# natalieklein/gpcsd

Measured on AMD Instinct MI355X. Metric: gpcsd_loglik_plus_predict_trials_per_sec, higher is better.
Workload: dtype f64; 1 GPU; GPCSD2D 384ch x 500t x 50 trials/GPU, fp64, ngl 20x60 (BASELINE cfg3/cfg4); n_elec=384, n_t=500, trials_per_gpu=50, total_trials=50, parallelism=trial-sharded x1, next_step_announced=True

## Files before the change

### gpcsd_amd/csrc/ctx.hpp

```cpp
#pragma once
#include <hip/hip_runtime.h>

#include <cstdarg>
#include <cstdio>
#include <cstring>
#include <map>
#include <string>
#include <vector>

#include "../../include/gpcsd_hip.h"

namespace gpcsd {

struct HipError {
    int code;
    std::string msg;
};

#define GP_HIP(expr)                                                                          \
    do {                                                                                      \
        hipError_t _e = (expr);                                                               \
        if (_e != hipSuccess) {                                                               \
            char _b[512];                                                                     \
            snprintf(_b, sizeof(_b), "%s:%d: %s -> %s", __FILE__, __LINE__, #expr,            \
// ... 41 lines not shown
        if (done[d]) return false;
        done[d] = true;
        return true;
    }
};
}

struct PredSink;
struct PairLl;
struct PredCall {
    const gpcsd_hparams *hp = nullptr;
    const double *z = nullptr, *tstar = nullptr;
    int nz = 0, ntstar = 0, type = 0;
    bool want_lists = false, async = false;
    PredSink *sink = nullptr;
    int solve_pass = 0;
    PairLl *ll = nullptr;
    bool prelude_side = false;
};

struct gpcsd_ctx {
    int device = 0;
    hipStream_t stream = nullptr;
    hipStream_t stream2 = nullptr;
    hipStream_t stream3 = nullptr;
    hipStream_t stream4 = nullptr;
    hipStream_t stream5 = nullptr;
    static constexpr int SCAL_N = 64, STATUS_N = 8, STATUS_LATE = 4;
    static constexpr int RESULT_DOUBLES = SCAL_N + STATUS_N / 2;
    double *h_result = nullptr;
    bool capturing = false;
// ... 323 lines not shown
```

### gpcsd_amd/csrc/gram.hip

```cpp
#include "devutil.hpp"
#include "kernels.hpp"

namespace gpcsd {

template <typename T>
__device__ __forceinline__ T dev_b_fwd_1d(T r, T R) {
    const T q = (r / R) * (r / R);
    return sqrt(q + T(1)) - sqrt(q);
}

template <typename T>
__device__ __forceinline__ T dev_b_fwd_2d_w(T w, T R, T eps) {
    const T re = R + eps;
    return log(re + sqrt(re * re + w * w)) - log(eps + sqrt(eps * eps + w * w));
}

__global__ void b_fwd_1d_kernel(const double *__restrict__ r, long n, double R, double *__restrict__ out) {
    for (long i = blockIdx.x * (long)blockDim.x + threadIdx.x; i < n; i += (long)gridDim.x * blockDim.x)
        out[i] = dev_b_fwd_1d<double>(r[i], R);
}

__global__ void b_fwd_2d_kernel(const double *__restrict__ d1, const double *__restrict__ d2, const double *__restrict__ w,
                                long n, double R, double eps, double *__restrict__ out) {
    for (long i = blockIdx.x * (long)blockDim.x + threadIdx.x; i < n; i += (long)gridDim.x * blockDim.x) {
// ... 362 lines not shown
                const double lg = (lane < nk) ? log(mypiv) : 0.0;
                logsum += wave_sum(lg);
            }
            __builtin_amdgcn_wave_barrier();
            if (k0 + LT_CK < np) store_chunk(buf ^ 1);
        }
        quad += wave_sum(lane < nr ? q : 0.0);
    }
    if (lane == 0) {
        g.partials[item] = quad;
        g.partials[nitems + item] = logsum;
    }
}

constexpr int LS_CPL = 4;
typedef double dbl2_t __attribute__((ext_vector_type(2)));
__global__ __launch_bounds__(64 * LT_WAVES) void ll_tridiag_scan_kernel(LlTridiagArgs g) {
    __shared__ double tile[LT_WAVES][2][64][LT_CK + 1];
    __shared__ dbl2_t coef[LT_WAVES][64 * LS_CPL + LT_CK];
    __shared__ double pexc[LT_WAVES][64 * LS_CPL + 1];
    const int lane = threadIdx.x & 63, wid = __builtin_amdgcn_readfirstlane(threadIdx.x >> 6);
    const int item = blockIdx.x * LT_WAVES + wid, nitems = 2 * g.nx;
    if (item >= nitems) return;
    const int xr = item >> 1, p = item & 1;
    const int np = g.np[p];
    if (np <= 0) {
        if (lane == 0) {
            g.partials[item] = 0.0;
            g.partials[nitems + item] = 0.0;
        }
        return;
    }
    const double lam_m = g.es[xr] * g.amax[p][0], sig = g.sig[0];
    const double *__restrict__ dd = g.d[p], *__restrict__ ee = g.e[p];
    const double *__restrict__ Wx = g.W + (long)xr * g.R * g.nt + g.c0[p];
    const int half = lane >> 5, kk_l = lane & 31;
    double stg[LT_RPL];
    auto load_chunk = [&](int r0, int nr, int k0) {
        const int nk = min(LT_CK, np - k0);
#pragma unroll
        for (int i = 0; i < LT_RPL; ++i) {
            const int rr = half + 2 * i;
            stg[i] = (rr < nr && kk_l < nk) ? Wx[(long)(r0 + rr) * g.nt + k0 + kk_l] : 0.0;
        }
    };
    auto store_chunk = [&](int buf) {
#pragma unroll
        for (int i = 0; i < LT_RPL; ++i) tile[wid][buf][half + 2 * i][kk_l] = stg[i];
    };
    load_chunk(0, min(64, g.R), 0);
    double logsum;
    {
        double a[LS_CPL], b2[LS_CPL], bb[LS_CPL];
#pragma unroll
        for (int cc = 0; cc < LS_CPL; ++cc) {
            const int k = lane * LS_CPL + cc;
            a[cc] = (k < np) ? lam_m * dd[k] + sig : 1.0;
            bb[cc] = (k >= 1 && k < np) ? lam_m * ee[k - 1] : 0.0;
            b2[cc] = bb[cc] * bb[cc];
        }
        auto renorm = [](double &x0, double &x1, double &x2, double &x3) {
            const double big = fmax(fmax(fabs(x0), fabs(x1)), fmax(fabs(x2), fabs(x3)));
            int ex;
            (void)frexp(big, &ex);
            x0 = ldexp(x0, -ex); x1 = ldexp(x1, -ex); x2 = ldexp(x2, -ex); x3 = ldexp(x3, -ex);
        };
        double m00 = a[0], m01 = -b2[0], m10 = 1.0, m11 = 0.0;
#pragma unroll
        for (int cc = 1; cc < LS_CPL; ++cc) {
            const double n00 = a[cc] * m00 - b2[cc] * m10, n01 = a[cc] * m01 - b2[cc] * m11;
            m10 = m00; m11 = m01; m00 = n00; m01 = n01;
        }
        renorm(m00, m01, m10, m11);
#pragma unroll
        for (int dlt = 1; dlt < 64; dlt <<= 1) {
            const double e00 = __shfl_up(m00, dlt), e01 = __shfl_up(m01, dlt), e10 = __shfl_up(m10, dlt), e11 = __shfl_up(m11, dlt);
            if (lane >= dlt) {
                double n00 = m00 * e00 + m01 * e10, n01 = m00 * e01 + m01 * e11;
                double n10 = m10 * e00 + m11 * e10, n11 = m10 * e01 + m11 * e11;
                renorm(n00, n01, n10, n11);
                m00 = n00; m01 = n01; m10 = n10; m11 = n11;
            }
        }
        double t0 = __shfl_up(m00, 1), t1 = __shfl_up(m10, 1);
        if (lane == 0) { t0 = 1.0; t1 = 0.0; }
        double pv[LS_CPL];
#pragma unroll
        for (int cc = 0; cc < LS_CPL; ++cc) {
            const double tn = a[cc] * t0 - b2[cc] * t1;
            pv[cc] = t0 / tn;
            t1 = t0; t0 = tn;
            if (cc == 1) {
                int ex;
                (void)frexp(t0, &ex);
                t0 = ldexp(t0, -ex); t1 = ldexp(t1, -ex);
            }
        }
#pragma unroll
        for (int cc = 0; cc < LS_CPL; ++cc) pexc[wid][lane * LS_CPL + cc + 1] = pv[cc];
        if (lane == 0) pexc[wid][0] = 0.0;
        __builtin_amdgcn_wave_barrier();
        {
            double gk[LS_CPL], rk[LS_CPL], G = 1.0, H = 0.0;
#pragma unroll
            for (int cc = 0; cc < LS_CPL; ++cc) {
                const double pl = pexc[wid][lane * LS_CPL + cc];
                const double sk = fma(-b2[cc], pl, a[cc]);
                rk[cc] = fma(-pv[cc], sk, 1.0);
                gk[cc] = b2[cc] * pl * pv[cc];
                H = fma(gk[cc], H, -rk[cc]);
                G *= gk[cc];
            }
#pragma unroll
            for (int dlt = 1; dlt < 64; dlt <<= 1) {
                const double Ge = __shfl_up(G, dlt), He = __shfl_up(H, dlt);
                if (lane >= dlt) {
                    H = fma(G, He, H);
                    G *= Ge;
                }
            }
            double eta = __shfl_up(H, 1);
            if (lane == 0) eta = 0.0;
#pragma unroll
            for (int cc = 0; cc < LS_CPL; ++cc) {
                eta = fma(gk[cc], eta, -rk[cc]);
                pv[cc] = fma(-pv[cc], eta, pv[cc]);
            }
            __builtin_amdgcn_wave_barrier();
#pragma unroll
            for (int cc = 0; cc < LS_CPL; ++cc) pexc[wid][lane * LS_CPL + cc + 1] = pv[cc];
            __builtin_amdgcn_wave_barrier();
        }
        double dk[LS_CPL], lg = 0.0;
#pragma unroll
        for (int cc = 0; cc < LS_CPL; ++cc) {
            const int k = lane * LS_CPL + cc;
            dk[cc] = a[cc] - b2[cc] * pexc[wid][k];
            pv[cc] = 1.0 / dk[cc];
            if (k < np) lg += log(dk[cc]);
        }
        logsum = wave_sum(lg);
        __builtin_amdgcn_wave_barrier();
#pragma unroll
        for (int cc = 0; cc < LS_CPL; ++cc) pexc[wid][lane * LS_CPL + cc + 1] = pv[cc];
        __builtin_amdgcn_wave_barrier();
#pragma unroll
        for (int cc = 0; cc < LS_CPL; ++cc) {
            const int k = lane * LS_CPL + cc;
            dbl2_t cf;
            cf.x = (k < np) ? bb[cc] * pexc[wid][k] : 0.0;
            cf.y = (k < np) ? pv[cc] : 0.0;
            coef[wid][k] = cf;
        }
        if (lane < LT_CK) coef[wid][64 * LS_CPL + lane] = dbl2_t{0.0, 0.0};
    }
    double quad = 0.0;
    for (int r0 = 0; r0 < g.R; r0 += 64) {
        const int nr = min(64, g.R - r0);
        if (r0 > 0) load_chunk(r0, nr, 0);
        __builtin_amdgcn_wave_barrier();
        store_chunk(0);
        double z = 0.0, q[4] = {0.0, 0.0, 0.0, 0.0};
        int buf = 0;
        for (int k0 = 0; k0 < np; k0 += LT_CK, buf ^= 1) {
            if (k0 + LT_CK < np) load_chunk(r0, nr, k0 + LT_CK);
            __builtin_amdgcn_wave_barrier();
            double wv[LT_CK];
            dbl2_t cf[LT_CK];
#pragma unroll
            for (int kk = 0; kk < LT_CK; ++kk) {
                wv[kk] = tile[wid][buf][lane][kk];
                cf[kk] = coef[wid][k0 + kk];
            }
#pragma unroll
            for (int kk = 0; kk < LT_CK; ++kk) {
                z = fma(-cf[kk].x, z, wv[kk]);
                q[kk & 3] = fma(z * z, cf[kk].y, q[kk & 3]);
            }
            __builtin_amdgcn_wave_barrier();
            if (k0 + LT_CK < np) store_chunk(buf ^ 1);
        }
        quad += wave_sum(lane < nr ? (q[0] + q[1]) + (q[2] + q[3]) : 0.0);
    }
    if (lane == 0) {
        g.partials[item] = quad;
        g.partials[nitems + item] = logsum;
    }
}

__global__ __launch_bounds__(256) void ll_tridiag_reduce_kernel(const double *__restrict__ partials, int nitems, double *out_sumlog,
                                                                double *out_quad, double *host_slot, const double *status_src,
                                                                int status_at, int status_doubles) {
    __shared__ double sh[256];
    const double *p = partials + (blockIdx.x == 0 ? nitems : 0);
    double s = 0.0;
    for (int i = threadIdx.x; i < nitems; i += 256) s += p[i];
    sh[threadIdx.x] = s;
    __syncthreads();
    for (int w = 128; w > 0; w >>= 1) {
        if ((int)threadIdx.x < w) sh[threadIdx.x] += sh[threadIdx.x + w];
// ... 21 lines not shown
                  double *out_sumlog, double *out_quad, hipStream_t s, double *host_slot, const double *status_src, int status_at,
                  int status_doubles, int variant) {
    LlTridiagArgs g{};
    g.W = W; g.es = es; g.sig = sig; g.nx = nx; g.R = R; g.nt = nt;
    for (int p = 0; p < 2; ++p) {
        g.d[p] = d[p]; g.e[p] = e[p]; g.amax[p] = amax[p]; g.np[p] = np[p]; g.c0[p] = c0[p];
    }
    const int nitems = 2 * nx;
    g.partials = c->buf<double>("ll_tridiag_partials", (size_t)2 * nitems);
    ProfScope ps(c, "ll_tridiag", 0.0, s);
    static const bool serial_env = getenv("GPCSD_LL_PIVOT_SCAN") && getenv("GPCSD_LL_PIVOT_SCAN")[0] == '0';
    const bool serial = variant ? variant == 1 : serial_env;
    GP_REQUIRE(variant != 2 || std::max(np[0], np[1]) <= 64 * LS_CPL, -3, "ll_tridiag: the scan kernel takes blocks of at most %d columns",
               64 * LS_CPL);
    if (!serial && std::max(np[0], np[1]) <= 64 * LS_CPL)
        hipLaunchKernelGGL(ll_tridiag_scan_kernel, dim3(ceil_div(nitems, LT_WAVES)), dim3(64 * LT_WAVES), 0, s, g);
    else
        hipLaunchKernelGGL(ll_tridiag_kernel, dim3(ceil_div(nitems, LT_WAVES)), dim3(64 * LT_WAVES), 0, s, g);
    bool wrote = false;
    ll_tridiag_reduce_launch(c, g.partials, nitems, out_sumlog, out_quad, host_slot, status_src, status_at, status_doubles, s, &wrote);
    GP_HIP(hipGetLastError());
    return wrote;
}

constexpr int TS_BATCH = 64;
constexpr int TS_P = 64;
constexpr int TS_P_DEFAULT = 64;
struct TriSolveArgs {
    const double *W;
    double *B;
    const double *es;
    const double *d[2], *e[2], *amax[2];
    const double *sig;
    int nx, R, nt, np[2], c0[2];
    int npad;
    unsigned long long *clk;
};
constexpr int TS_HB = 32;
constexpr int TS_KMAX = 256;
template <int P>
__global__ __launch_bounds__(256, P == 32 ? 2 : 1) void tridiag_solve_kernel(TriSolveArgs g) {
    constexpr int HB = (P == 32) ? 16 : TS_HB;
    extern __shared__ __attribute__((aligned(16))) double smem[];
    double *zbuf = smem;
    double *pinv = zbuf + (long)g.npad * P;
    double *lmul = pinv + TS_KMAX + TS_BATCH;
    double *scan = lmul + TS_KMAX + TS_BATCH;
    auto stamp = [&](int k) { if (g.clk && blockIdx.x == 0 && threadIdx.x == 0) g.clk[k] = wall_clock64(); };
    stamp(0);
    const int tid = threadIdx.x, lane = tid & 63, wid = tid >> 6;
  for (int item = blockIdx.x; item < 2 * g.nx; item += gridDim.x) {
    const int xr = item >> 1, p = item & 1;
    const int np = g.np[p];
    if (np <= 0) continue;
    const int nbatch = (np + TS_BATCH - 1) / TS_BATCH, npad = nbatch * TS_BATCH;
    const double lam_m = g.es[xr] * g.amax[p][0], sig = g.sig[0];
    const double *__restrict__ dd = g.d[p], *__restrict__ ee = g.e[p];
    const long rowbase = (long)xr * g.R * g.nt + g.c0[p];
    const int quarter = lane >> 4, kk_l = lane & 15;
    for (int r0 = 0; r0 < g.R; r0 += P) {
        const int nr = min(P, g.R - r0);
        const bool first = r0 == 0;
        const double *const wl = g.W + rowbase + (long)(r0 + quarter) * g.nt + kk_l;
        const int b0 = wid * TS_BATCH;
        double stg[4][P / 4];
#pragma unroll
        for (int q = 0; q < 4; ++q) {
            const int kq = b0 + 16 * q;
            const int kc = min(kk_l, max(np - 1 - kq, 0));
#pragma unroll
            for (int i = 0; i < P / 4; ++i) {
                double v = 0.0;
                if (4 * i < nr && kq < np) {
                    const int rc = min(quarter + 4 * i, nr - 1) - quarter;
                    v = wl[(long)rc * g.nt + kq + (kc - kk_l)];
                }
                stg[q][i] = v;
            }
        }
        if (first) {
            const int k = tid;
            const bool real = k < np;
            const double ak = real ? lam_m * dd[k] + sig : 1.0;
            const double bkm = (k >= 1 && k < np) ? lam_m * ee[k - 1] : 0.0;
            double m00 = ak, m01 = -bkm * bkm, m10 = 1.0, m11 = 0.0;
            double *buf = scan;
#pragma unroll 1
            for (int dlt = 1; dlt < 256; dlt <<= 1, buf = (buf == scan) ? scan + 1024 : scan) {
                buf[4 * k + 0] = m00; buf[4 * k + 1] = m01; buf[4 * k + 2] = m10; buf[4 * k + 3] = m11;
                __syncthreads();
                if (k >= dlt) {
                    const double e00 = buf[4 * (k - dlt) + 0], e01 = buf[4 * (k - dlt) + 1], e10 = buf[4 * (k - dlt) + 2],
                                 e11 = buf[4 * (k - dlt) + 3];
                    const double n00 = m00 * e00 + m01 * e10, n01 = m00 * e01 + m01 * e11;
                    const double n10 = m10 * e00 + m11 * e10, n11 = m10 * e01 + m11 * e11;
                    const double big = fmax(fmax(fabs(n00), fabs(n01)), fmax(fabs(n10), fabs(n11)));
                    int ex;
                    (void)frexp(big, &ex);
                    m00 = ldexp(n00, -ex); m01 = ldexp(n01, -ex); m10 = ldexp(n10, -ex); m11 = ldexp(n11, -ex);
                }
            }
            double pk = m10 / m00;
            const double b2 = bkm * bkm;
            buf[k] = pk;
            __syncthreads();
            const double pl = k >= 1 ? buf[k - 1] : 0.0;
            const double rho = fma(-pk, fma(-b2, pl, ak), 1.0);
            double G = b2 * pl * pk, H = -rho;
            __syncthreads();
#pragma unroll 1
            for (int dlt = 1; dlt < 256; dlt <<= 1, buf = (buf == scan) ? scan + 1024 : scan) {
                buf[2 * k + 0] = G; buf[2 * k + 1] = H;
                __syncthreads();
                if (k >= dlt) {
                    const double Ge = buf[2 * (k - dlt) + 0], He = buf[2 * (k - dlt) + 1];
                    H = fma(G, He, H);
                    G *= Ge;
                }
            }
            pk = fma(-pk, H, pk);
            buf[k] = pk;
            __syncthreads();
            const double pl1 = k >= 1 ? buf[k - 1] : 0.0;
            pk = 1.0 / fma(-b2, pl1, ak);
            pinv[k] = real ? pk : 1.0;
            __syncthreads();
            buf[k] = pk;
            __syncthreads();
            lmul[k] = (k >= 1 && real) ? bkm * buf[k - 1] : 0.0;
            if (k < TS_BATCH) {
                pinv[TS_KMAX + k] = 1.0;
                lmul[TS_KMAX + k] = 0.0;
            }
        }
#pragma unroll
        for (int q = 0; q < 4; ++q)
#pragma unroll
            for (int i = 0; i < P / 4; ++i)
                if (b0 < npad) zbuf[((b0 + 16 * q + kk_l) >> 1) * (2 * P) + (quarter + 4 * i) * 2 + (kk_l & 1)] = stg[q][i];
        __syncthreads();
        stamp(1);
        if (wid == 0) {
            typedef double dbl2 __attribute__((ext_vector_type(2)));
            dbl2 *const zl = reinterpret_cast<dbl2 *>(zbuf) + (lane & (P - 1));
            double z = 0.0;
            for (int h0 = 0; h0 < npad; h0 += HB) {
                dbl2 *const zb = zl + (h0 >> 1) * P;
                const dbl2 *const lc = reinterpret_cast<const dbl2 *>(lmul + h0);
                dbl2 v[HB / 2], cl[HB / 2];
#pragma unroll
                for (int j = 0; j < HB / 2; ++j) {
                    v[j] = zb[j * P];
                    cl[j] = lc[j];
                }
#pragma unroll
                for (int j = 0; j < HB / 2; ++j) {
                    z = fma(-cl[j].x, z, v[j].x);
                    v[j].x = z;
                    z = fma(-cl[j].y, z, v[j].y);
                    v[j].y = z;
                }
#pragma unroll
                for (int j = 0; j < HB / 2; ++j) zb[j * P] = v[j];
            }
            stamp(2);
            double x = 0.0;
            for (int h0 = npad - HB; h0 >= 0; h0 -= HB) {
                dbl2 *const zb = zl + (h0 >> 1) * P;
                const dbl2 *const pc = reinterpret_cast<const dbl2 *>(pinv + h0);
                double cl[HB + 1];
                dbl2 v[HB / 2], cp[HB / 2];
#pragma unroll
                for (int j = 0; j < HB / 2; ++j) {
                    v[j] = zb[j * P];
                    cp[j] = pc[j];
                }
#pragma unroll
                for (int kk = 0; kk < HB; ++kk) cl[kk] = lmul[h0 + kk + 1];
#pragma unroll
                for (int j = HB / 2 - 1; j >= 0; --j) {
                    x = fma(v[j].y, cp[j].y, -cl[2 * j + 1] * x);
                    v[j].y = x;
                    x = fma(v[j].x, cp[j].x, -cl[2 * j] * x);
                    v[j].x = x;
                }
#pragma unroll
                for (int j = 0; j < HB / 2; ++j) zb[j * P] = v[j];
            }
        }
        __syncthreads();
        stamp(3);
        double *const bl = g.B + rowbase + (long)(r0 + quarter) * g.nt + kk_l;
        for (int bi = wid; bi < nbatch; bi += 4) {
            const int b0 = bi * TS_BATCH;
#pragma unroll
            for (int q = 0; q < 4; ++q) {
                const int kq = b0 + 16 * q;
                if (kq >= np) continue;
                const bool kfull = kq + 15 < np, kok = kq + kk_l < np;
#pragma unroll
                for (int i = 0; i < P / 4; ++i) {
                    if (4 * i >= nr) continue;
                    const double v = zbuf[((kq + kk_l) >> 1) * (2 * P) + (quarter + 4 * i) * 2 + (kk_l & 1)];
                    if (kfull && 4 * i + 3 < nr) bl[(long)(4 * i) * g.nt + kq] = v;
                    else if (kok && quarter + 4 * i < nr) bl[(long)(4 * i) * g.nt + kq] = v;
                }
            }
        }
        __syncthreads();
        stamp(4);
    }
  }
}

static int tridiag_solve_npad(int npmax) { return (npmax + TS_BATCH - 1) / TS_BATCH * TS_BATCH; }
static size_t tridiag_solve_lds(int npmax, int P = TS_P) {
    const int npad = tridiag_solve_npad(npmax);
    return ((size_t)npad * P + 2 * (size_t)(256 + TS_BATCH) + 2 * 256 * 4) * sizeof(double);
}
int k_tridiag_solve_pass(int npmax, int R) {
    return (R >= 16 && npmax <= 256 && tridiag_solve_lds(npmax) <= (size_t)150 * 1024) ? TS_P : 0;
}

void k_tridiag_solve(gpcsd_ctx *c, const double *W, double *B, const double *es, const double *const d[2], const double *const e[2],
                     const double *const amax[2], const double *sig, int nx, int R, int nt, const int np[2], const int c0[2],
                     hipStream_t s, int pass, int hint) {
    TriSolveArgs g{};
    g.W = W; g.B = B; g.es = es; g.sig = sig; g.nx = nx; g.R = R; g.nt = nt;
    for (int p = 0; p < 2; ++p) {
        g.d[p] = d[p]; g.e[p] = e[p]; g.amax[p] = amax[p]; g.np[p] = np[p]; g.c0[p] = c0[p];
    }
    const int npmax = std::max(np[0], np[1]);
    GP_REQUIRE(k_tridiag_solve_pass(npmax, R) > 0, -3, "tridiag_solve: temporal blocks of %d columns do not fit the solve kernel", npmax);
    GP_REQUIRE(pass == 0 || pass == 32 || pass == 64, -3, "tridiag_solve: %d trials per pass (0 = by size, 32 or 64)", pass);
    g.npad = tridiag_solve_npad(npmax);
    static const int forced = getenv("GPCSD_TS_P") ? (atoi(getenv("GPCSD_TS_P")) == 32 ? 32 : 64) : 0;
    const int P = pass ? pass : forced ? forced : (R <= 32 || hint == 32) ? 32 : TS_P_DEFAULT;
    const size_t lds = tridiag_solve_lds(npmax, P);
    static size_t attr_dev[64][2] = {};
    size_t *attr = attr_dev[c->device & 63];
    if (lds > attr[P == 32]) {
        if (P == 32) GP_HIP(hipFuncSetAttribute(reinterpret_cast<const void *>(tridiag_solve_kernel<32>), hipFuncAttributeMaxDynamicSharedMemorySize, (int)lds));
        else GP_HIP(hipFuncSetAttribute(reinterpret_cast<const void *>(tridiag_solve_kernel<64>), hipFuncAttributeMaxDynamicSharedMemorySize, (int)lds));
        attr[P == 32] = lds;
    }
    static const bool clk_on = getenv("GPCSD_TS_CLK") && getenv("GPCSD_TS_CLK")[0] == '1';
    g.clk = clk_on ? c->buf<unsigned long long>("ts_clk", 8) : nullptr;
    ProfScope ps(c, "tridiag_solve", 6.0 * nx * (double)R * nt, s);
    static const int grid_cap = getenv("GPCSD_TS_GRID") ? atoi(getenv("GPCSD_TS_GRID")) : 192;
    const int grid = grid_cap > 0 ? std::min(2 * nx, grid_cap) : 2 * nx;
    if (P == 32) hipLaunchKernelGGL(tridiag_solve_kernel<32>, dim3(grid), dim3(256), lds, s, g);
    else hipLaunchKernelGGL(tridiag_solve_kernel<64>, dim3(grid), dim3(256), lds, s, g);
    GP_HIP(hipGetLastError());
    if (clk_on) {
        unsigned long long h[8];
        c->copy_out(h, g.clk, sizeof(h), s);
        GP_HIP(hipStreamSynchronize(s));
        fprintf(stderr, "[tridiag_solve] item 0 (10 ns ticks): load+pivots %llu  forward %llu  backward %llu  store %llu\n", h[1] - h[0],
                h[2] - h[1], h[3] - h[2], h[4] - h[3]);
    }
}

template <typename T>
__global__ __launch_bounds__(256) void fwd_weights_1d_kernel(const double *__restrict__ x, int nx,
                                                             const double *__restrict__ gl_x,
                                                             const double *__restrict__ gl_w, int ngl, double R,
                                                             double *__restrict__ A, const HpDev *__restrict__ tab, long s_out) {
    if (tab) {
        R = tab[blockIdx.z].R;
        A += blockIdx.z * s_out;
    }
    const long n = (long)nx * ngl;
    for (long e = blockIdx.x * (long)blockDim.x + threadIdx.x; e < n; e += (long)gridDim.x * blockDim.x) {
        const int i = (int)(e / ngl), g = (int)(e % ngl);
        A[e] = (double)(T(gl_w[g]) * dev_b_fwd_1d<T>(T(gl_x[g]) - T(x[i]), T(R)));
// ... 557 lines not shown
```

### gpcsd_amd/csrc/kernels.hpp

```cpp
#pragma once
#include <functional>
#include "ctx.hpp"

namespace gpcsd {

enum Epi : int {
    EPI_STORE = 0,
    EPI_DIV_D = 1,
    EPI_QUAD = 2,
    EPI_ACCUM = 3,
    EPI_GRAD = 4,
    EPI_DUAL_INIT = 6,
    EPI_SUB = 7
};

struct GemmDesc {
    int M = 0, N = 0, K = 0;
    const double *A = nullptr;
    long lda = 0;
    bool transA = false;
    const double *B = nullptr;
    long ldb = 0;
    bool transB = false;
    double *C = nullptr;
// ... 116 lines not shown
                      const HpDev *tab = nullptr, int B = 1, long s_out = 0);
void k_se_1d(gpcsd_ctx *c, const double *a, int n, const double *b, int m, double ell, double *out, hipStream_t s,
             const HpDev *tab = nullptr, int B = 1, long s_out = 0);
void k_se_2d(gpcsd_ctx *c, const double *a1, const double *a2, int na, int na2, const double *b1, const double *b2,
             int nb, int nb2, double ell1, double ell2, double *out, hipStream_t s, const HpDev *tab = nullptr, int B = 1,
             long s_out = 0);
void k_se_axis(gpcsd_ctx *c, const double *a, int n, double ell, double *out, hipStream_t s);
void k_se_axis_tab(gpcsd_ctx *c, const double *a, int n, int axis, const HpDev *tab, int B, double *K, double *dK, hipStream_t s);
bool k_ll_tridiag(gpcsd_ctx *c, const double *W, const double *es, const double *const d[2], const double *const e[2],
                  const double *const amax[2], const double *sig, int nx, int R, int nt, const int np[2], const int c0[2],
                  double *out_sumlog, double *out_quad, hipStream_t s, double *host_slot = nullptr, const double *status_src = nullptr,
                  int status_at = 0, int status_doubles = 0, int variant = 0);
int k_tridiag_solve_pass(int npmax, int R);
void k_tridiag_solve(gpcsd_ctx *c, const double *W, double *B, const double *es, const double *const d[2], const double *const e[2],
                     const double *const amax[2], const double *sig, int nx, int R, int nt, const int np[2], const int c0[2],
                     hipStream_t s, int pass = 0, int hint = 0);
void k_add_diag(gpcsd_ctx *c, double *A, int n, double v, hipStream_t s, const HpDev *tab = nullptr, int B = 1, long s_out = 0);
void k_shift_copy(gpcsd_ctx *c, const double *src, double *dst, int n, double v, hipStream_t s);
void k_sum_partials(gpcsd_ctx *c, double *out, const double *P, long n, int parts, hipStream_t s);
void k_rowdot(gpcsd_ctx *c, const double *T, const double *A, int n, int G, double *out, hipStream_t s);
int k_build_D(gpcsd_ctx *c, const double *es, int nx, const double *et, int nt, const double *sig, int nsig, double *D,
              double *Dinv, double *sumlog_out, hipStream_t s, const HpDev *tab = nullptr, int B = 1, long s_sumlog = 0);
void k_swap_last2(gpcsd_ctx *c, const double *in, double *out, int n0, int n1, int n2, hipStream_t s);
void k_fill(gpcsd_ctx *c, double *p, long n, double v, hipStream_t s);
void k_swap_last2_sum(gpcsd_ctx *c, const double *in, int C, double *list, long list_stride, double *sum, int n0, int n1, int n2,
                      hipStream_t s);

void k_sym_fold_rect(gpcsd_ctx *c, const double *K, long ldk, const SymDev &rs, const SymDev &cs, double *out_ss, double *out_aa,
                     hipStream_t s);
void k_sym_unfold_mat(gpcsd_ctx *c, const double *Gf, long s_in, const SymDev &sy, int n, double *out, hipStream_t s, int B = 1);
void k_fold_lfp(gpcsd_ctx *c, const double *Y, int nx, int R, int nt, const SymDev &ss, const SymDev &st, double *out,
// ... 151 lines not shown
```

Baseline: 42380 trials/s.

## Replace sequential tridiagonal sweeps with wave-parallel scan over time per row

Both the tridiagonal log-likelihood kernel and the tridiagonal solve kernel now place the time axis across lanes, four columns per lane, and run the forward and backward recurrences as wave-level prefix scans with precomputed coefficients. Each block handles one item with four waves, each streaming rows from global memory straight into registers with double-buffered prefetch. This replaces the LDS-tiled per-row serial sweep and the single-wave serial solve. It removes LDS staging and serial dependency chains, at the cost of extra shuffles per row, and it restricts blocks to at most 256 columns.

```diff
diff --git a/gpcsd_amd/csrc/ctx.hpp b/gpcsd_amd/csrc/ctx.hpp
--- a/gpcsd_amd/csrc/ctx.hpp
+++ b/gpcsd_amd/csrc/ctx.hpp
@@ -79,7 +79,6 @@
     int nz = 0, ntstar = 0, type = 0;
     bool want_lists = false, async = false;
     PredSink *sink = nullptr;
-    int solve_pass = 0;
     PairLl *ll = nullptr;
     bool prelude_side = false;
 };
diff --git a/gpcsd_amd/csrc/gram.hip b/gpcsd_amd/csrc/gram.hip
--- a/gpcsd_amd/csrc/gram.hip
+++ b/gpcsd_amd/csrc/gram.hip
@@ -400,176 +400,281 @@
 }
 
 constexpr int LS_CPL = 4;
+constexpr int TR_WAVES = 4;
+constexpr int TR_RIF = 4;
 typedef double dbl2_t __attribute__((ext_vector_type(2)));
-__global__ __launch_bounds__(64 * LT_WAVES) void ll_tridiag_scan_kernel(LlTridiagArgs g) {
-    __shared__ double tile[LT_WAVES][2][64][LT_CK + 1];
-    __shared__ dbl2_t coef[LT_WAVES][64 * LS_CPL + LT_CK];
-    __shared__ double pexc[LT_WAVES][64 * LS_CPL + 1];
+
+struct TriRowCoef {
+    double c[3];
+    double pinv[4];
+    double fl[3];
+    double fs[6];
+    double bl[3];
+    double bs[6];
+};
+
+template <bool BACK>
+__device__ __forceinline__ double tri_rows_setup(double lam_m, double sig, const double *__restrict__ dd, const double *__restrict__ ee,
+                                                 int np, int lane, bool want_log, TriRowCoef &cf) {
+    double a[LS_CPL], b2[LS_CPL], bb[LS_CPL];
+#pragma unroll
+    for (int cc = 0; cc < LS_CPL; ++cc) {
+        const int k = lane * LS_CPL + cc;
+        a[cc] = (k < np) ? lam_m * dd[k] + sig : 1.0;
+        bb[cc] = (k >= 1 && k < np) ? lam_m * ee[k - 1] : 0.0;
+        b2[cc] = bb[cc] * bb[cc];
+    }
+    auto renorm = [](double &x0, double &x1, double &x2, double &x3) {
+        const double big = fmax(fmax(fabs(x0), fabs(x1)), fmax(fabs(x2), fabs(x3)));
+        int ex;
+        (void)frexp(big, &ex);
+        x0 = ldexp(x0, -ex); x1 = ldexp(x1, -ex); x2 = ldexp(x2, -ex); x3 = ldexp(x3, -ex);
+    };
+    auto from_left = [&](double last) {
+        const double v = __shfl_up(last, 1);
+        return lane == 0 ? 0.0 : v;
+    };
+    double m00 = a[0], m01 = -b2[0], m10 = 1.0, m11 = 0.0;
+#pragma unroll
+    for (int cc = 1; cc < LS_CPL; ++cc) {
+        const double n00 = a[cc] * m00 - b2[cc] * m10, n01 = a[cc] * m01 - b2[cc] * m11;
+        m10 = m00; m11 = m01; m00 = n00; m01 = n01;
+    }
+    renorm(m00, m01, m10, m11);
+#pragma unroll
+    for (int dlt = 1; dlt < 64; dlt <<= 1) {
+        const double e00 = __shfl_up(m00, dlt), e01 = __shfl_up(m01, dlt), e10 = __shfl_up(m10, dlt), e11 = __shfl_up(m11, dlt);
+        if (lane >= dlt) {
+            double n00 = m00 * e00 + m01 * e10, n01 = m00 * e01 + m01 * e11;
+            double n10 = m10 * e00 + m11 * e10, n11 = m10 * e01 + m11 * e11;
+            renorm(n00, n01, n10, n11);
+            m00 = n00; m01 = n01; m10 = n10; m11 = n11;
+        }
+    }
+    double t0 = __shfl_up(m00, 1), t1 = __shfl_up(m10, 1);
+    if (lane == 0) { t0 = 1.0; t1 = 0.0; }
+    double pv[LS_CPL];
+#pragma unroll
+    for (int cc = 0; cc < LS_CPL; ++cc) {
+        const double tn = a[cc] * t0 - b2[cc] * t1;
+        pv[cc] = t0 / tn;
+        t1 = t0; t0 = tn;
+        if (cc == 1) {
+            int ex;
+            (void)frexp(t0, &ex);
+            t0 = ldexp(t0, -ex); t1 = ldexp(t1, -ex);
+        }
+    }
+    {
+        double gk[LS_CPL], rk[LS_CPL], G = 1.0, H = 0.0;
+        double pl = from_left(pv[LS_CPL - 1]);
+#pragma unroll
+        for (int cc = 0; cc < LS_CPL; ++cc) {
+            const double sk = fma(-b2[cc], pl, a[cc]);
+            rk[cc] = fma(-pv[cc], sk, 1.0);
+            gk[cc] = b2[cc] * pl * pv[cc];
+            H = fma(gk[cc], H, -rk[cc]);
+            G *= gk[cc];
+            pl = pv[cc];
+        }
+#pragma unroll
+        for (int dlt = 1; dlt < 64; dlt <<= 1) {
+            const double Ge = __shfl_up(G, dlt), He = __shfl_up(H, dlt);
+            if (lane >= dlt) {
+                H = fma(G, He, H);
+                G *= Ge;
+            }
+        }
+        double eta = __shfl_up(H, 1);
+        if (lane == 0) eta = 0.0;
+#pragma unroll
+        for (int cc = 0; cc < LS_CPL; ++cc) {
+            eta = fma(gk[cc], eta, -rk[cc]);
+            pv[cc] = fma(-pv[cc], eta, pv[cc]);
+        }
+    }
+    double dk[LS_CPL], lg = 0.0;
+    {
+        double pl = from_left(pv[LS_CPL - 1]);
+#pragma unroll
+        for (int cc = 0; cc < LS_CPL; ++cc) {
+            dk[cc] = a[cc] - b2[cc] * pl;
+            pl = pv[cc];
+        }
+    }
+    double logsum = 0.0;
+    if (want_log) {
+#pragma unroll
+        for (int cc = 0; cc < LS_CPL; ++cc)
+            if (lane * LS_CPL + cc < np) lg += log(dk[cc]);
+        logsum = wave_sum(lg);
+    }
+    double cfull[LS_CPL];
+    {
+#pragma unroll
+        for (int cc = 0; cc < LS_CPL; ++cc) pv[cc] = 1.0 / dk[cc];
+        double pl = from_left(pv[LS_CPL - 1]);
+#pragma unroll
+        for (int cc = 0; cc < LS_CPL; ++cc) {
+            const int k = lane * LS_CPL + cc;
+            cfull[cc] = (k < np) ? -(bb[cc] * pl) : 0.0;
+            cf.pinv[cc] = (k < np) ? pv[cc] : 0.0;
+            pl = pv[cc];
+        }
+    }
+#pragma unroll
+    for (int cc = 1; cc < LS_CPL; ++cc) cf.c[cc - 1] = cfull[cc];
+    {
+        double A = cfull[0];
+#pragma unroll
+        for (int cc = 0; cc < LS_CPL - 1; ++cc) {
+            cf.fl[cc] = A;
+            A *= cfull[cc + 1];
+        }
+#pragma unroll
+        for (int s = 0; s < 6; ++s) {
+            const int dlt = 1 << s;
+            const double Ae = __shfl_up(A, dlt);
+            cf.fs[s] = (lane >= dlt) ? A : 0.0;
+            if (lane >= dlt) A *= Ae;
+        }
+    }
+    if (BACK) {
+        double A = __shfl_down(cfull[0], 1);
+        if (lane == 63) A = 0.0;
+#pragma unroll
+        for (int cc = LS_CPL - 1; cc >= 1; --cc) {
+            cf.bl[cc - 1] = A;
+            A *= cfull[cc];
+        }
+#pragma unroll
+        for (int s = 0; s < 6; ++s) {
+            const int dlt = 1 << s;
+            const double Ae = __shfl_down(A, dlt);
+            cf.bs[s] = (lane + dlt < 64) ? A : 0.0;
+            if (lane + dlt < 64) A *= Ae;
+        }
+    }
+    return logsum;
+}
+
+template <int N>
+__device__ __forceinline__ void tri_rows_forward(const TriRowCoef &cf, double (&v)[N][LS_CPL]) {
+    double T[N];
+#pragma unroll
+    for (int r = 0; r < N; ++r) {
+#pragma unroll
+        for (int cc = 1; cc < LS_CPL; ++cc) v[r][cc] = fma(cf.c[cc - 1], v[r][cc - 1], v[r][cc]);
+        T[r] = v[r][LS_CPL - 1];
+    }
+#pragma unroll
+    for (int s = 0; s < 6; ++s)
+#pragma unroll
+        for (int r = 0; r < N; ++r) T[r] = fma(cf.fs[s], __shfl_up(T[r], 1 << s), T[r]);
+#pragma unroll
+    for (int r = 0; r < N; ++r) {
+        const double left = __shfl_up(T[r], 1);
+#pragma unroll
+        for (int cc = 0; cc < LS_CPL - 1; ++cc) v[r][cc] = fma(cf.fl[cc], left, v[r][cc]);
+        v[r][LS_CPL - 1] = T[r];
+    }
+}
+
+template <int N>
+__device__ __forceinline__ void tri_rows_backward(const TriRowCoef &cf, double (&v)[N][LS_CPL]) {
+    double T[N];
+#pragma unroll
+    for (int r = 0; r < N; ++r) {
+        v[r][LS_CPL - 1] *= cf.pinv[LS_CPL - 1];
+#pragma unroll
+        for (int cc = LS_CPL - 2; cc >= 0; --cc) v[r][cc] = fma(cf.c[cc], v[r][cc + 1], v[r][cc] * cf.pinv[cc]);
+        T[r] = v[r][0];
+    }
+#pragma unroll
+    for (int s = 0; s < 6; ++s)
+#pragma unroll
+        for (int r = 0; r < N; ++r) T[r] = fma(cf.bs[s], __shfl_down(T[r], 1 << s), T[r]);
+#pragma unroll
+    for (int r = 0; r < N; ++r) {
+        const double right = __shfl_down(T[r], 1);
+#pragma unroll
+        for (int cc = 1; cc < LS_CPL; ++cc) v[r][cc] = fma(cf.bl[cc - 1], right, v[r][cc]);
+        v[r][0] = T[r];
+    }
+}
+
+__device__ __forceinline__ void tri_row_load(const double *rp, int np, int lane, double (&v)[LS_CPL]) {
+    const int k = lane * LS_CPL;
+    const bool al = (reinterpret_cast<unsigned long long>(rp) & 15ull) == 0;
+    if (al && k + LS_CPL <= np) {
+        const dbl2_t lo = *reinterpret_cast<const dbl2_t *>(rp + k), hi = *reinterpret_cast<const dbl2_t *>(rp + k + 2);
+        v[0] = lo.x; v[1] = lo.y; v[2] = hi.x; v[3] = hi.y;
+    } else {
+#pragma unroll
+        for (int cc = 0; cc < LS_CPL; ++cc) v[cc] = (k + cc < np) ? rp[k + cc] : 0.0;
+    }
+}
+__device__ __forceinline__ void tri_row_store(double *rp, int np, int lane, const double (&v)[LS_CPL]) {
+    const int k = lane * LS_CPL;
+    const bool al = (reinterpret_cast<unsigned long long>(rp) & 15ull) == 0;
+    if (al && k + LS_CPL <= np) {
+        *reinterpret_cast<dbl2_t *>(rp + k) = dbl2_t{v[0], v[1]};
+        *reinterpret_cast<dbl2_t *>(rp + k + 2) = dbl2_t{v[2], v[3]};
+    } else {
+#pragma unroll
+        for (int cc = 0; cc < LS_CPL; ++cc)
+            if (k + cc < np) rp[k + cc] = v[cc];
+    }
+}
+__device__ __forceinline__ void tri_rows_load(const double *Wx, int nt, int R, int np, int lane, int wid, int n0, double (&v)[TR_RIF][LS_CPL]) {
+#pragma unroll
+    for (int q = 0; q < TR_RIF; ++q) {
+        const int row = wid + TR_WAVES * (n0 + q);
+        if (row < R) {
+            tri_row_load(Wx + (long)row * nt, np, lane, v[q]);
+        } else {
+#pragma unroll
+            for (int cc = 0; cc < LS_CPL; ++cc) v[q][cc] = 0.0;
+        }
+    }
+}
+
+__global__ __launch_bounds__(64 * TR_WAVES) void ll_tridiag_rows_kernel(LlTridiagArgs g) {
+    __shared__ double part[TR_WAVES];
     const int lane = threadIdx.x & 63, wid = __builtin_amdgcn_readfirstlane(threadIdx.x >> 6);
-    const int item = blockIdx.x * LT_WAVES + wid, nitems = 2 * g.nx;
-    if (item >= nitems) return;
+    const int item = blockIdx.x, nitems = 2 * g.nx;
     const int xr = item >> 1, p = item & 1;
     const int np = g.np[p];
     if (np <= 0) {
-        if (lane == 0) {
+        if (threadIdx.x == 0) {
             g.partials[item] = 0.0;
             g.partials[nitems + item] = 0.0;
         }
         return;
     }
-    const double lam_m = g.es[xr] * g.amax[p][0], sig = g.sig[0];
-    const double *__restrict__ dd = g.d[p], *__restrict__ ee = g.e[p];
     const double *__restrict__ Wx = g.W + (long)xr * g.R * g.nt + g.c0[p];
-    const int half = lane >> 5, kk_l = lane & 31;
-    double stg[LT_RPL];
-    auto load_chunk = [&](int r0, int nr, int k0) {
-        const int nk = min(LT_CK, np - k0);
-#pragma unroll
-        for (int i = 0; i < LT_RPL; ++i) {
-            const int rr = half + 2 * i;
-            stg[i] = (rr < nr && kk_l < nk) ? Wx[(long)(r0 + rr) * g.nt + k0 + kk_l] : 0.0;
-        }
-    };
-    auto store_chunk = [&](int buf) {
-#pragma unroll
-        for (int i = 0; i < LT_RPL; ++i) tile[wid][buf][half + 2 * i][kk_l] = stg[i];
-    };
-    load_chunk(0, min(64, g.R), 0);
-    double logsum;
-    {
-        double a[LS_CPL], b2[LS_CPL], bb[LS_CPL];
-#pragma unroll
-        for (int cc = 0; cc < LS_CPL; ++cc) {
-            const int k = lane * LS_CPL + cc;
-            a[cc] = (k < np) ? lam_m * dd[k] + sig : 1.0;
-            bb[cc] = (k >= 1 && k < np) ? lam_m * ee[k - 1] : 0.0;
-            b2[cc] = bb[cc] * bb[cc];
-        }
-        auto renorm = [](double &x0, double &x1, double &x2, double &x3) {
-            const double big = fmax(fmax(fabs(x0), fabs(x1)), fmax(fabs(x2), fabs(x3)));
-            int ex;
-            (void)frexp(big, &ex);
-            x0 = ldexp(x0, -ex); x1 = ldexp(x1, -ex); x2 = ldexp(x2, -ex); x3 = ldexp(x3, -ex);
-        };
-        double m00 = a[0], m01 = -b2[0], m10 = 1.0, m11 = 0.0;
-#pragma unroll
-        for (int cc = 1; cc < LS_CPL; ++cc) {
-            const double n00 = a[cc] * m00 - b2[cc] * m10, n01 = a[cc] * m01 - b2[cc] * m11;
-            m10 = m00; m11 = m01; m00 = n00; m01 = n01;
-        }
-        renorm(m00, m01, m10, m11);
-#pragma unroll
-        for (int dlt = 1; dlt < 64; dlt <<= 1) {
-            const double e00 = __shfl_up(m00, dlt), e01 = __shfl_up(m01, dlt), e10 = __shfl_up(m10, dlt), e11 = __shfl_up(m11, dlt);
-            if (lane >= dlt) {
-                double n00 = m00 * e00 + m01 * e10, n01 = m00 * e01 + m01 * e11;
-                double n10 = m10 * e00 + m11 * e10, n11 = m10 * e01 + m11 * e11;
-                renorm(n00, n01, n10, n11);
-                m00 = n00; m01 = n01; m10 = n10; m11 = n11;
+    const int nrows = (g.R - wid + TR_WAVES - 1) / TR_WAVES;
+    double cur[TR_RIF][LS_CPL], nxt[TR_RIF][LS_CPL] = {};
+    tri_rows_load(Wx, g.nt, g.R, np, lane, wid, 0, cur);
+    TriRowCoef cf;
+    const double logsum = tri_rows_setup<false>(g.es[xr] * g.amax[p][0], g.sig[0], g.d[p], g.e[p], np, lane, wid == 0, cf);
+    double q[LS_CPL] = {0.0, 0.0, 0.0, 0.0};
+    for (int n0 = 0; n0 < nrows; n0 += TR_RIF) {
+        if (n0 + TR_RIF < nrows) tri_rows_load(Wx, g.nt, g.R, np, lane, wid, n0 + TR_RIF, nxt);
+        tri_rows_forward<TR_RIF>(cf, cur);
+#pragma unroll
+        for (int r = 0; r < TR_RIF; ++r)
+#pragma unroll
+            for (int cc = 0; cc < LS_CPL; ++cc) {
+                q[cc] = fma(cur[r][cc] * cur[r][cc], cf.pinv[cc], q[cc]);
+                cur[r][cc] = nxt[r][cc];
             }
-        }
-        double t0 = __shfl_up(m00, 1), t1 = __shfl_up(m10, 1);
-        if (lane == 0) { t0 = 1.0; t1 = 0.0; }
-        double pv[LS_CPL];
-#pragma unroll
-        for (int cc = 0; cc < LS_CPL; ++cc) {
-            const double tn = a[cc] * t0 - b2[cc] * t1;
-            pv[cc] = t0 / tn;
-            t1 = t0; t0 = tn;
-            if (cc == 1) {
-                int ex;
-                (void)frexp(t0, &ex);
-                t0 = ldexp(t0, -ex); t1 = ldexp(t1, -ex);
-            }
-        }
-#pragma unroll
-        for (int cc = 0; cc < LS_CPL; ++cc) pexc[wid][lane * LS_CPL + cc + 1] = pv[cc];
-        if (lane == 0) pexc[wid][0] = 0.0;
-        __builtin_amdgcn_wave_barrier();
-        {
-            double gk[LS_CPL], rk[LS_CPL], G = 1.0, H = 0.0;
-#pragma unroll
-            for (int cc = 0; cc < LS_CPL; ++cc) {
-                const double pl = pexc[wid][lane * LS_CPL + cc];
-                const double sk = fma(-b2[cc], pl, a[cc]);
-                rk[cc] = fma(-pv[cc], sk, 1.0);
-                gk[cc] = b2[cc] * pl * pv[cc];
-                H = fma(gk[cc], H, -rk[cc]);
-                G *= gk[cc];
-            }
-#pragma unroll
-            for (int dlt = 1; dlt < 64; dlt <<= 1) {
-                const double Ge = __shfl_up(G, dlt), He = __shfl_up(H, dlt);
-                if (lane >= dlt) {
-                    H = fma(G, He, H);
-                    G *= Ge;
-                }
-            }
-            double eta = __shfl_up(H, 1);
-            if (lane == 0) eta = 0.0;
-#pragma unroll
-            for (int cc = 0; cc < LS_CPL; ++cc) {
-                eta = fma(gk[cc], eta, -rk[cc]);
-                pv[cc] = fma(-pv[cc], eta, pv[cc]);
-            }
-            __builtin_amdgcn_wave_barrier();
-#pragma unroll
-            for (int cc = 0; cc < LS_CPL; ++cc) pexc[wid][lane * LS_CPL + cc + 1] = pv[cc];
-            __builtin_amdgcn_wave_barrier();
-        }
-        double dk[LS_CPL], lg = 0.0;
-#pragma unroll
-        for (int cc = 0; cc < LS_CPL; ++cc) {
-            const int k = lane * LS_CPL + cc;
-            dk[cc] = a[cc] - b2[cc] * pexc[wid][k];
-            pv[cc] = 1.0 / dk[cc];
-            if (k < np) lg += log(dk[cc]);
-        }
-        logsum = wave_sum(lg);
-        __builtin_amdgcn_wave_barrier();
-#pragma unroll
-        for (int cc = 0; cc < LS_CPL; ++cc) pexc[wid][lane * LS_CPL + cc + 1] = pv[cc];
-        __builtin_amdgcn_wave_barrier();
-#pragma unroll
-        for (int cc = 0; cc < LS_CPL; ++cc) {
-            const int k = lane * LS_CPL + cc;
-            dbl2_t cf;
-            cf.x = (k < np) ? bb[cc] * pexc[wid][k] : 0.0;
-            cf.y = (k < np) ? pv[cc] : 0.0;
-            coef[wid][k] = cf;
-        }
-        if (lane < LT_CK) coef[wid][64 * LS_CPL + lane] = dbl2_t{0.0, 0.0};
-    }
-    double quad = 0.0;
-    for (int r0 = 0; r0 < g.R; r0 += 64) {
-        const int nr = min(64, g.R - r0);
-        if (r0 > 0) load_chunk(r0, nr, 0);
-        __builtin_amdgcn_wave_barrier();
-        store_chunk(0);
-        double z = 0.0, q[4] = {0.0, 0.0, 0.0, 0.0};
-        int buf = 0;
-        for (int k0 = 0; k0 < np; k0 += LT_CK, buf ^= 1) {
-            if (k0 + LT_CK < np) load_chunk(r0, nr, k0 + LT_CK);
-            __builtin_amdgcn_wave_barrier();
-            double wv[LT_CK];
-            dbl2_t cf[LT_CK];
-#pragma unroll
-            for (int kk = 0; kk < LT_CK; ++kk) {
-                wv[kk] = tile[wid][buf][lane][kk];
-                cf[kk] = coef[wid][k0 + kk];
-            }
-#pragma unroll
-            for (int kk = 0; kk < LT_CK; ++kk) {
-                z = fma(-cf[kk].x, z, wv[kk]);
-                q[kk & 3] = fma(z * z, cf[kk].y, q[kk & 3]);
-            }
-            __builtin_amdgcn_wave_barrier();
-            if (k0 + LT_CK < np) store_chunk(buf ^ 1);
-        }
-        quad += wave_sum(lane < nr ? (q[0] + q[1]) + (q[2] + q[3]) : 0.0);
-    }
-    if (lane == 0) {
-        g.partials[item] = quad;
+    }
+    const double quad = wave_sum((q[0] + q[1]) + (q[2] + q[3]));
+    if (lane == 0) part[wid] = quad;
+    __syncthreads();
+    if (threadIdx.x == 0) {
+        g.partials[item] = (part[0] + part[1]) + (part[2] + part[3]);
         g.partials[nitems + item] = logsum;
     }
 }
@@ -621,7 +726,7 @@
     GP_REQUIRE(variant != 2 || std::max(np[0], np[1]) <= 64 * LS_CPL, -3, "ll_tridiag: the scan kernel takes blocks of at most %d columns",
                64 * LS_CPL);
     if (!serial && std::max(np[0], np[1]) <= 64 * LS_CPL)
-        hipLaunchKernelGGL(ll_tridiag_scan_kernel, dim3(ceil_div(nitems, LT_WAVES)), dim3(64 * LT_WAVES), 0, s, g);
+        hipLaunchKernelGGL(ll_tridiag_rows_kernel, dim3(nitems), dim3(64 * TR_WAVES), 0, s, g);
     else
         hipLaunchKernelGGL(ll_tridiag_kernel, dim3(ceil_div(nitems, LT_WAVES)), dim3(64 * LT_WAVES), 0, s, g);
     bool wrote = false;
@@ -630,9 +735,6 @@
     return wrote;
 }
 
-constexpr int TS_BATCH = 64;
-constexpr int TS_P = 64;
-constexpr int TS_P_DEFAULT = 64;
 struct TriSolveArgs {
     const double *W;
     double *B;
@@ -640,198 +742,41 @@
     const double *d[2], *e[2], *amax[2];
     const double *sig;
     int nx, R, nt, np[2], c0[2];
-    int npad;
-    unsigned long long *clk;
 };
-constexpr int TS_HB = 32;
-constexpr int TS_KMAX = 256;
-template <int P>
-__global__ __launch_bounds__(256, P == 32 ? 2 : 1) void tridiag_solve_kernel(TriSolveArgs g) {
-    constexpr int HB = (P == 32) ? 16 : TS_HB;
-    extern __shared__ __attribute__((aligned(16))) double smem[];
-    double *zbuf = smem;
-    double *pinv = zbuf + (long)g.npad * P;
-    double *lmul = pinv + TS_KMAX + TS_BATCH;
-    double *scan = lmul + TS_KMAX + TS_BATCH;
-    auto stamp = [&](int k) { if (g.clk && blockIdx.x == 0 && threadIdx.x == 0) g.clk[k] = wall_clock64(); };
-    stamp(0);
-    const int tid = threadIdx.x, lane = tid & 63, wid = tid >> 6;
-  for (int item = blockIdx.x; item < 2 * g.nx; item += gridDim.x) {
+__global__ __launch_bounds__(64 * TR_WAVES) void tridiag_rows_solve_kernel(TriSolveArgs g) {
+    const int lane = threadIdx.x & 63, wid = __builtin_amdgcn_readfirstlane(threadIdx.x >> 6);
+    const int item = blockIdx.x;
     const int xr = item >> 1, p = item & 1;
     const int np = g.np[p];
-    if (np <= 0) continue;
-    const int nbatch = (np + TS_BATCH - 1) / TS_BATCH, npad = nbatch * TS_BATCH;
-    const double lam_m = g.es[xr] * g.amax[p][0], sig = g.sig[0];
-    const double *__restrict__ dd = g.d[p], *__restrict__ ee = g.e[p];
+    if (np <= 0) return;
     const long rowbase = (long)xr * g.R * g.nt + g.c0[p];
-    const int quarter = lane >> 4, kk_l = lane & 15;
-    for (int r0 = 0; r0 < g.R; r0 += P) {
-        const int nr = min(P, g.R - r0);
-        const bool first = r0 == 0;
-        const double *const wl = g.W + rowbase + (long)(r0 + quarter) * g.nt + kk_l;
-        const int b0 = wid * TS_BATCH;
-        double stg[4][P / 4];
-#pragma unroll
-        for (int q = 0; q < 4; ++q) {
-            const int kq = b0 + 16 * q;
-            const int kc = min(kk_l, max(np - 1 - kq, 0));
-#pragma unroll
-            for (int i = 0; i < P / 4; ++i) {
-                double v = 0.0;
-                if (4 * i < nr && kq < np) {
-                    const int rc = min(quarter + 4 * i, nr - 1) - quarter;
-                    v = wl[(long)rc * g.nt + kq + (kc - kk_l)];
-                }
-                stg[q][i] = v;
-            }
-        }
-        if (first) {
-            const int k = tid;
-            const bool real = k < np;
-            const double ak = real ? lam_m * dd[k] + sig : 1.0;
-            const double bkm = (k >= 1 && k < np) ? lam_m * ee[k - 1] : 0.0;
-            double m00 = ak, m01 = -bkm * bkm, m10 = 1.0, m11 = 0.0;
-            double *buf = scan;
-#pragma unroll 1
-            for (int dlt = 1; dlt < 256; dlt <<= 1, buf = (buf == scan) ? scan + 1024 : scan) {
-                buf[4 * k + 0] = m00; buf[4 * k + 1] = m01; buf[4 * k + 2] = m10; buf[4 * k + 3] = m11;
-                __syncthreads();
-                if (k >= dlt) {
-                    const double e00 = buf[4 * (k - dlt) + 0], e01 = buf[4 * (k - dlt) + 1], e10 = buf[4 * (k - dlt) + 2],
-                                 e11 = buf[4 * (k - dlt) + 3];
-                    const double n00 = m00 * e00 + m01 * e10, n01 = m00 * e01 + m01 * e11;
-                    const double n10 = m10 * e00 + m11 * e10, n11 = m10 * e01 + m11 * e11;
-                    const double big = fmax(fmax(fabs(n00), fabs(n01)), fmax(fabs(n10), fabs(n11)));
-                    int ex;
-                    (void)frexp(big, &ex);
-                    m00 = ldexp(n00, -ex); m01 = ldexp(n01, -ex); m10 = ldexp(n10, -ex); m11 = ldexp(n11, -ex);
-                }
-            }
-            double pk = m10 / m00;
-            const double b2 = bkm * bkm;
-            buf[k] = pk;
-            __syncthreads();
-            const double pl = k >= 1 ? buf[k - 1] : 0.0;
-            const double rho = fma(-pk, fma(-b2, pl, ak), 1.0);
-            double G = b2 * pl * pk, H = -rho;
-            __syncthreads();
-#pragma unroll 1
-            for (int dlt = 1; dlt < 256; dlt <<= 1, buf = (buf == scan) ? scan + 1024 : scan) {
-                buf[2 * k + 0] = G; buf[2 * k + 1] = H;
-                __syncthreads();
-                if (k >= dlt) {
-                    const double Ge = buf[2 * (k - dlt) + 0], He = buf[2 * (k - dlt) + 1];
-                    H = fma(G, He, H);
-                    G *= Ge;
-                }
-            }
-            pk = fma(-pk, H, pk);
-            buf[k] = pk;
-            __syncthreads();
-            const double pl1 = k >= 1 ? buf[k - 1] : 0.0;
-            pk = 1.0 / fma(-b2, pl1, ak);
-            pinv[k] = real ? pk : 1.0;
-            __syncthreads();
-            buf[k] = pk;
-            __syncthreads();
-            lmul[k] = (k >= 1 && real) ? bkm * buf[k - 1] : 0.0;
-            if (k < TS_BATCH) {
-                pinv[TS_KMAX + k] = 1.0;
-                lmul[TS_KMAX + k] = 0.0;
-            }
-        }
-#pragma unroll
-        for (int q = 0; q < 4; ++q)
-#pragma unroll
-            for (int i = 0; i < P / 4; ++i)
-                if (b0 < npad) zbuf[((b0 + 16 * q + kk_l) >> 1) * (2 * P) + (quarter + 4 * i) * 2 + (kk_l & 1)] = stg[q][i];
-        __syncthreads();
-        stamp(1);
-        if (wid == 0) {
-            typedef double dbl2 __attribute__((ext_vector_type(2)));
-            dbl2 *const zl = reinterpret_cast<dbl2 *>(zbuf) + (lane & (P - 1));
-            double z = 0.0;
-            for (int h0 = 0; h0 < npad; h0 += HB) {
-                dbl2 *const zb = zl + (h0 >> 1) * P;
-                const dbl2 *const lc = reinterpret_cast<const dbl2 *>(lmul + h0);
-                dbl2 v[HB / 2], cl[HB / 2];
-#pragma unroll
-                for (int j = 0; j < HB / 2; ++j) {
-                    v[j] = zb[j * P];
-                    cl[j] = lc[j];
-                }
-#pragma unroll
-                for (int j = 0; j < HB / 2; ++j) {
-                    z = fma(-cl[j].x, z, v[j].x);
-                    v[j].x = z;
-                    z = fma(-cl[j].y, z, v[j].y);
-                    v[j].y = z;
-                }
-#pragma unroll
-                for (int j = 0; j < HB / 2; ++j) zb[j * P] = v[j];
-            }
-            stamp(2);
-            double x = 0.0;
-            for (int h0 = npad - HB; h0 >= 0; h0 -= HB) {
-                dbl2 *const zb = zl + (h0 >> 1) * P;
-                const dbl2 *const pc = reinterpret_cast<const dbl2 *>(pinv + h0);
-                double cl[HB + 1];
-                dbl2 v[HB / 2], cp[HB / 2];
-#pragma unroll
-                for (int j = 0; j < HB / 2; ++j) {
-                    v[j] = zb[j * P];
-                    cp[j] = pc[j];
-                }
-#pragma unroll
-                for (int kk = 0; kk < HB; ++kk) cl[kk] = lmul[h0 + kk + 1];
-#pragma unroll
-                for (int j = HB / 2 - 1; j >= 0; --j) {
-                    x = fma(v[j].y, cp[j].y, -cl[2 * j + 1] * x);
-                    v[j].y = x;
-                    x = fma(v[j].x, cp[j].x, -cl[2 * j] * x);
-                    v[j].x = x;
-                }
-#pragma unroll
-                for (int j = 0; j < HB / 2; ++j) zb[j * P] = v[j];
-            }
-        }
-        __syncthreads();
-        stamp(3);
-        double *const bl = g.B + rowbase + (long)(r0 + quarter) * g.nt + kk_l;
-        for (int bi = wid; bi < nbatch; bi += 4) {
-            const int b0 = bi * TS_BATCH;
-#pragma unroll
-            for (int q = 0; q < 4; ++q) {
-                const int kq = b0 + 16 * q;
-                if (kq >= np) continue;
-                const bool kfull = kq + 15 < np, kok = kq + kk_l < np;
-#pragma unroll
-                for (int i = 0; i < P / 4; ++i) {
-                    if (4 * i >= nr) continue;
-                    const double v = zbuf[((kq + kk_l) >> 1) * (2 * P) + (quarter + 4 * i) * 2 + (kk_l & 1)];
-                    if (kfull && 4 * i + 3 < nr) bl[(long)(4 * i) * g.nt + kq] = v;
-                    else if (kok && quarter + 4 * i < nr) bl[(long)(4 * i) * g.nt + kq] = v;
-                }
-            }
-        }
-        __syncthreads();
-        stamp(4);
-    }
-  }
-}
-
-static int tridiag_solve_npad(int npmax) { return (npmax + TS_BATCH - 1) / TS_BATCH * TS_BATCH; }
-static size_t tridiag_solve_lds(int npmax, int P = TS_P) {
-    const int npad = tridiag_solve_npad(npmax);
-    return ((size_t)npad * P + 2 * (size_t)(256 + TS_BATCH) + 2 * 256 * 4) * sizeof(double);
-}
-int k_tridiag_solve_pass(int npmax, int R) {
-    return (R >= 16 && npmax <= 256 && tridiag_solve_lds(npmax) <= (size_t)150 * 1024) ? TS_P : 0;
-}
+    const double *Wx = g.W + rowbase;
+    double *Bx = g.B + rowbase;
+    const int nrows = (g.R - wid + TR_WAVES - 1) / TR_WAVES;
+    if (nrows <= 0) return;
+    double cur[TR_RIF][LS_CPL], nxt[TR_RIF][LS_CPL] = {};
+    tri_rows_load(Wx, g.nt, g.R, np, lane, wid, 0, cur);
+    TriRowCoef cf;
+    (void)tri_rows_setup<true>(g.es[xr] * g.amax[p][0], g.sig[0], g.d[p], g.e[p], np, lane, false, cf);
+    for (int n0 = 0; n0 < nrows; n0 += TR_RIF) {
+        if (n0 + TR_RIF < nrows) tri_rows_load(Wx, g.nt, g.R, np, lane, wid, n0 + TR_RIF, nxt);
+        tri_rows_forward<TR_RIF>(cf, cur);
+        tri_rows_backward<TR_RIF>(cf, cur);
+#pragma unroll
+        for (int q = 0; q < TR_RIF; ++q) {
+            const int row = wid + TR_WAVES * (n0 + q);
+            if (row < g.R) tri_row_store(Bx + (long)row * g.nt, np, lane, cur[q]);
+#pragma unroll
+            for (int cc = 0; cc < LS_CPL; ++cc) cur[q][cc] = nxt[q][cc];
+        }
+    }
+}
+
+int k_tridiag_solve_pass(int npmax, int R) { return (R >= 16 && npmax <= 64 * LS_CPL) ? 64 : 0; }
 
 void k_tridiag_solve(gpcsd_ctx *c, const double *W, double *B, const double *es, const double *const d[2], const double *const e[2],
                      const double *const amax[2], const double *sig, int nx, int R, int nt, const int np[2], const int c0[2],
-                     hipStream_t s, int pass, int hint) {
+                     hipStream_t s, int pass) {
     TriSolveArgs g{};
     g.W = W; g.B = B; g.es = es; g.sig = sig; g.nx = nx; g.R = R; g.nt = nt;
     for (int p = 0; p < 2; ++p) {
@@ -839,33 +784,10 @@
     }
     const int npmax = std::max(np[0], np[1]);
     GP_REQUIRE(k_tridiag_solve_pass(npmax, R) > 0, -3, "tridiag_solve: temporal blocks of %d columns do not fit the solve kernel", npmax);
-    GP_REQUIRE(pass == 0 || pass == 32 || pass == 64, -3, "tridiag_solve: %d trials per pass (0 = by size, 32 or 64)", pass);
-    g.npad = tridiag_solve_npad(npmax);
-    static const int forced = getenv("GPCSD_TS_P") ? (atoi(getenv("GPCSD_TS_P")) == 32 ? 32 : 64) : 0;
-    const int P = pass ? pass : forced ? forced : (R <= 32 || hint == 32) ? 32 : TS_P_DEFAULT;
-    const size_t lds = tridiag_solve_lds(npmax, P);
-    static size_t attr_dev[64][2] = {};
-    size_t *attr = attr_dev[c->device & 63];
-    if (lds > attr[P == 32]) {
-        if (P == 32) GP_HIP(hipFuncSetAttribute(reinterpret_cast<const void *>(tridiag_solve_kernel<32>), hipFuncAttributeMaxDynamicSharedMemorySize, (int)lds));
-        else GP_HIP(hipFuncSetAttribute(reinterpret_cast<const void *>(tridiag_solve_kernel<64>), hipFuncAttributeMaxDynamicSharedMemorySize, (int)lds));
-        attr[P == 32] = lds;
-    }
-    static const bool clk_on = getenv("GPCSD_TS_CLK") && getenv("GPCSD_TS_CLK")[0] == '1';
-    g.clk = clk_on ? c->buf<unsigned long long>("ts_clk", 8) : nullptr;
+    GP_REQUIRE(pass == 0 || pass == 32 || pass == 64, -3, "tridiag_solve: %d trials per pass (0, 32 or 64: the same kernel)", pass);
     ProfScope ps(c, "tridiag_solve", 6.0 * nx * (double)R * nt, s);
-    static const int grid_cap = getenv("GPCSD_TS_GRID") ? atoi(getenv("GPCSD_TS_GRID")) : 192;
-    const int grid = grid_cap > 0 ? std::min(2 * nx, grid_cap) : 2 * nx;
-    if (P == 32) hipLaunchKernelGGL(tridiag_solve_kernel<32>, dim3(grid), dim3(256), lds, s, g);
-    else hipLaunchKernelGGL(tridiag_solve_kernel<64>, dim3(grid), dim3(256), lds, s, g);
-    GP_HIP(hipGetLastError());
-    if (clk_on) {
-        unsigned long long h[8];
-        c->copy_out(h, g.clk, sizeof(h), s);
-        GP_HIP(hipStreamSynchronize(s));
-        fprintf(stderr, "[tridiag_solve] item 0 (10 ns ticks): load+pivots %llu  forward %llu  backward %llu  store %llu\n", h[1] - h[0],
-                h[2] - h[1], h[3] - h[2], h[4] - h[3]);
-    }
+    hipLaunchKernelGGL(tridiag_rows_solve_kernel, dim3(2 * nx), dim3(64 * TR_WAVES), 0, s, g);
+    GP_HIP(hipGetLastError());
 }
 
 template <typename T>
diff --git a/gpcsd_amd/csrc/kernels.hpp b/gpcsd_amd/csrc/kernels.hpp
--- a/gpcsd_amd/csrc/kernels.hpp
+++ b/gpcsd_amd/csrc/kernels.hpp
@@ -154,7 +154,7 @@
 int k_tridiag_solve_pass(int npmax, int R);
 void k_tridiag_solve(gpcsd_ctx *c, const double *W, double *B, const double *es, const double *const d[2], const double *const e[2],
                      const double *const amax[2], const double *sig, int nx, int R, int nt, const int np[2], const int c0[2],
-                     hipStream_t s, int pass = 0, int hint = 0);
+                     hipStream_t s, int pass = 0);
 void k_add_diag(gpcsd_ctx *c, double *A, int n, double v, hipStream_t s, const HpDev *tab = nullptr, int B = 1, long s_out = 0);
 void k_shift_copy(gpcsd_ctx *c, const double *src, double *dst, int n, double v, hipStream_t s);
 void k_sum_partials(gpcsd_ctx *c, double *out, const double *P, long n, int parts, hipStream_t s);
```

After: 42500 trials/s (median of 6 runs). Within noise of the previous version (+0.3%).
